# VITA-Group/mm-hand

Hardware: AMD Instinct MI355X
Metric: 256x256 hand images/sec (G+D step) (higher is better)
Workload: dtype f32; 1 GPU; RHD-shaped 256x256, per-GPU batch 32, fp32 (Winograd F(6x6,3x3) on the 3x3 stack), G(9 PATBlocks, ngf64)+D_PB+D_PP+L1/perceptual/GAN+Adam, --norm instance, dropout on; VGG19[:4] weights: random-init (seed 1234): NOT the reference's pretrained objective; global_batch=32, parallelism=dp1

## Files before the change

### include/mmhand_hip.h

```cpp
#ifndef MMHAND_HIP_H
#define MMHAND_HIP_H

#include <stddef.h>
#include <stdint.h>

#ifdef __cplusplus
extern "C" {
#endif
#pragma GCC visibility push(default)

typedef void* mmh_stream_t;

enum { MMH_PAD_ZERO = 0, MMH_PAD_REFLECT = 1 };
enum { MMH_ACT_NONE = 0, MMH_ACT_RELU = 1, MMH_ACT_TANH = 2 };
enum { MMH_F32 = 0, MMH_BF16 = 1, MMH_FP16 = 2 };

typedef struct mmh_conv_desc {
    int32_t B, H, W;
    int32_t Cin, Cout;
    int32_t kh, kw;
    int32_t stride;
    int32_t pad;
    int32_t pad_mode;
    int32_t Ho, Wo;
    int32_t x_cs, y_cs;
    int32_t dtype;
} mmh_conv_desc;

const char* mmh_last_error(void);
int mmh_version(void);
int mmh_set_option(const char* key, int value);
int mmh_get_option(const char* key, int* value);
const char* mmh_option_key(int index);


int mmh_conv2d_fprop(const mmh_conv_desc* d, const void* x, const void* w,
                     const void* bias, void* y, int act, mmh_stream_t s);

int mmh_conv2d_fprop_stats_chunks(const mmh_conv_desc* d);
int mmh_conv2d_fprop_stats(const mmh_conv_desc* d, const void* x, const void* w, const void* bias,
                           void* y, void* stats, mmh_stream_t s);
int mmh_dgrad_s2_halo_supported(const mmh_conv_desc* d, int dx_cs);

int mmh_conv2d_dgrad(const mmh_conv_desc* d, const void* dy, const void* w,
                     void* dx, int dx_cs, mmh_stream_t s);

size_t mmh_conv2d_dgrad_folded_ws_bytes(const mmh_conv_desc* d);
int mmh_conv2d_dgrad_folded(const mmh_conv_desc* d, const void* dy, const void* w,
                            void* dx, void* ws, size_t ws_bytes, mmh_stream_t s);

int mmh_wino_weights(const void* w, int Cin, int Cout, int flip_transpose, int tile, int dtype,
                     void* U, mmh_stream_t s);
int mmh_wino_input(const void* x, int B, int H, int W, int C, int reflect, int tile, int dtype,
                   void* V, mmh_stream_t s);
int mmh_wino_dy(const void* dy, int B, int H, int W, int C, int tile, int dtype, void* Yh,
                mmh_stream_t s);
int mmh_wino_input_dy(const void* dy, int B, int H, int W, int C, int tile, int dtype, void* V,
                      void* Yh, int fold, mmh_stream_t s);
int mmh_wino_gemm(const void* V, const void* U, void* M, int64_t tiles, int K, int N,
                  int nbatch, int dtype, mmh_stream_t s);
int mmh_wino_gemm_levels(const void* V, const void* U, void* M, int64_t tiles, int K, int N,
                         int nbatch, int levels, mmh_stream_t s);
int mmh_wino_gemm_levels16(const void* V, const void* U, void* M, int64_t tiles, int K, int N, int levels,
                           mmh_stream_t s);
int mmh_wino_weights_multi(const void* table, int n, int64_t total_blocks, mmh_stream_t s);
int mmh_wino_output(const void* M, void* y, const void* bias, int B, int H, int W, int C,
                    int act, int tile, int dtype, void* stats, int fold, mmh_stream_t s);
size_t mmh_wino_wgrad_gemm_ws_bytes(int64_t tiles, int Cin, int Cout, int nbatch);
int mmh_wino_wgrad_gemm(const void* V, const void* Yh, int64_t tiles, int Cin, int Cout,
                        int nbatch, int dtype, void* ws, size_t ws_bytes, void* dU,
                        mmh_stream_t s);
int mmh_wino_dw(const void* dU, int Cin, int Cout, int tile, void* dw, int accumulate,
                mmh_stream_t s);
size_t mmh_conv2d_dgrad_border_ws_bytes(const mmh_conv_desc* d);
int mmh_conv2d_dgrad_border(const mmh_conv_desc* d, const void* dy, const void* w, void* dx,
                            void* ws, size_t ws_bytes, int phase, int io16, mmh_stream_t s);

size_t mmh_conv2d_wgrad_ws_bytes(const mmh_conv_desc* d);
int mmh_conv2d_wgrad(const mmh_conv_desc* d, const void* x, const void* dy,
                     void* dw, void* ws, size_t ws_bytes, int accumulate,
                     int io16, mmh_stream_t s);

int mmh_convT2d_fprop(const mmh_conv_desc* d, const void* x, const void* w,
                      const void* bias, void* y, int y_cs, int act,
                      mmh_stream_t s);
int mmh_convT2d_dgrad(const mmh_conv_desc* d, const void* dy, const void* w,
                      void* dx, mmh_stream_t s);
int mmh_convT2d_wgrad(const mmh_conv_desc* d, const void* x, const void* dy,
                      void* dw, void* ws, size_t ws_bytes, int accumulate,
                     int io16, mmh_stream_t s);

int mmh_prep_weights_bf16(const void* w, int taps, int Cin, int Cout,
                          void* w_plain, void* w_t, mmh_stream_t s);
int mmh_prep_weights_fp16(const void* w, int taps, int Cin, int Cout,
                          void* w_plain, void* w_t, mmh_stream_t s);
// ... 438 lines not shown
```

### mmhand_amd/csrc/common.h

```cpp
#pragma once
#include <hip/hip_runtime.h>
#include <cstdarg>
#include <cstdio>
#include <cstdint>
#include "../../include/mmhand_hip.h"

namespace mmh {

char* err_buf();
int fail(const char* fmt, ...);

inline int check_launch(const char* what) {
    hipError_t e = hipGetLastError();
    if (e != hipSuccess) return fail("%s: %s", what, hipGetErrorString(e));
    return 0;
}

inline hipStream_t as_stream(mmh_stream_t s) { return reinterpret_cast<hipStream_t>(s); }

inline int64_t cdiv(int64_t a, int64_t b) { return (a + b - 1) / b; }

int wino6_weights(const float* w, float* U, int Cin, int Cout, int flip_transpose, hipStream_t st);
int wino6_weights_multi(const long long* table, int n, long long total_blocks, hipStream_t st);
int wino6_input(const float* x, float* V, int B, int H, int W, int C, int reflect, int xcd, hipStream_t st);
int wino6_output(const float* M, float* y, const float* bias, int B, int H, int W, int C, int act, float* stats,
                 int fold, hipStream_t st);
int wino6_dy(const float* dy, float* Yh, int B, int H, int W, int C, hipStream_t st);
int wino6_input_normact(const float* x, float* V, int B, int H, int W, int C, int reflect, int xcd,
                        const float* scale, const float* shift, int groups, int relu, float drop_p,
                        const uint32_t* drows, hipStream_t st);
int wino6_input_dy_normbwd(const float* g, const float* x, float* V, float* Yh, int B, int H, int W, int C, int xcd,
                           int fold, const float* mean, const float* invstd, const float* gamma, const float* s1,
                           const float* s2, double count, const float* scale, const float* shift,
                           const uint32_t* drows, int groups, int relu, float drop_p, hipStream_t st);
int wino6_input_dy(const float* dy, float* V, float* Yh, int B, int H, int W, int C, int xcd, int fold,
                   hipStream_t st);
int wino6_dw(const float* dU, float* dw, int Cin, int Cout, int accumulate, hipStream_t st);
bool wgrad_lp16t_supported(const mmh_conv_desc* d);
int wgrad_lp16t_splits(const mmh_conv_desc* d);
int launch_wgrad_lp16t(const mmh_conv_desc* d, const void* x16, const void* dy16, float* slab, const void* zeros,
                       hipStream_t st);
bool dgrad_s2_halo_ok(const mmh_conv_desc* d, int dx_cs, int act);
int launch_dgrad_s2_halo(const mmh_conv_desc* d, const void* dy, const void* w, const void* bias, void* dx, int dx_cs,
                         int act, hipStream_t st);
extern int g_dgrad_s2_halo, g_dgrad_s2_dbg;
bool wgrad_s2_strip_ok(const mmh_conv_desc* d);
size_t wgrad_s2_strip_ws_bytes(const mmh_conv_desc* d);
int launch_wgrad_s2_strip(const mmh_conv_desc* d, const void* x, const void* dy, void* dw, void* ws, size_t ws_bytes,
                          int accumulate, hipStream_t st);
extern int g_wgrad_s2_strip;
bool stem_f32_ok(const mmh_conv_desc* d);
int stem_f32_stats_chunks(const mmh_conv_desc* d);
int launch_stem_f32(const mmh_conv_desc* d, const void* x, const void* w, const void* bias, void* y, int act, float* stats,
                    hipStream_t st);
extern int g_stem_f32, g_stem_f32_dbg, g_stem_f32_levels;
extern int g_stem_sparse;
extern int g_stem_sparse_flat;
void wgrad_flat_split(int Mrows, int N, int P, int& splits, int& pix_per_split);
bool wino_wgrad_dma_ok(int64_t tiles, int Cin, int Cout, int nbatch);
size_t wino_wgrad_dma_ws_bytes(int64_t tiles, int Cin, int Cout, int nbatch);
int launch_wino_wgrad_dma(const float* V, const float* Yh, int64_t tiles, int Cin, int Cout, int nbatch, float* ws, float* dU,
                          hipStream_t st);
extern int g_wino_wgrad_dma;
int launch_slab_reduce(const float* slab, float* dw, int64_t n4_total, int splits, int accumulate, int64_t n4, hipStream_t st);
bool conv_s2f_ok(const mmh_conv_desc* d, int mode);
bool conv_s1f_ok(const mmh_conv_desc* d, int mode);
int conv_s2f_stats_chunks(const mmh_conv_desc* d);
int launch_conv_s2f(const mmh_conv_desc* d, const void* x16, const void* w16, const void* bias, void* y, int y_is16, int act,
                    const void* zeros, hipStream_t st, float* stats = nullptr, int mode = 0);
bool conv_s2d_ok(const mmh_conv_desc* d, int mode);
int launch_conv_s2d(const mmh_conv_desc* d, const void* g16, const void* w16, const void* bias, void* dx, int dx_is16, int act,
                    const void* zeros, hipStream_t st);
extern int g_lp16_s2f;
extern int g_lp16_persist;
extern int g_slab_reduce_par;
extern int g_wino6_vec;
extern int g_lp16_shape;
extern int g_lp16_tap_inner;
extern int g_lp16_dbg;
extern int g_lp16_wgrad_ring;
extern int g_lp16_wgrad_s2;
extern int g_pw_v2;
extern int g_col_chunks, g_row_chunks;

}

#define MMH_REQUIRE(cond, ...)                      \
    do {                                            \
        if (!(cond)) return mmh::fail(__VA_ARGS__); \
    } while (0)
```

### mmhand_amd/csrc/conv_igemm.hip

```cpp
#include <algorithm>
#include <cstring>
#include "device_prims.h"

namespace {
using namespace mmh::dev;

typedef __bf16 bf16x4 __attribute__((ext_vector_type(4)));
typedef __bf16 bf16x2 __attribute__((ext_vector_type(2)));
typedef _Float16 f16x4 __attribute__((ext_vector_type(4)));
typedef _Float16 f16x2 __attribute__((ext_vector_type(2)));
__device__ __forceinline__ bf16x4 to_bf16x4(float4 v) {
    bf16x4 r;
    r[0] = (__bf16)v.x; r[1] = (__bf16)v.y; r[2] = (__bf16)v.z; r[3] = (__bf16)v.w;
    return r;
}
template <bool H16>
__device__ __forceinline__ bf16x4 to_lp4(float4 v) {
    if (H16) {
        f16x4 r;
        r[0] = (_Float16)v.x; r[1] = (_Float16)v.y; r[2] = (_Float16)v.z; r[3] = (_Float16)v.w;
        return __builtin_bit_cast(bf16x4, r);
    }
    return to_bf16x4(v);
}
template <int LP>
__device__ __forceinline__ void wst4(void* base, long long idx4, float4 v) {
    if (LP) reinterpret_cast<bf16x4*>(base)[idx4] = to_lp4<LP == 2>(v);
    else reinterpret_cast<float4*>(base)[idx4] = v;
}
template <int LP>
__device__ __forceinline__ float4 wld4(const void* base, long long idx4) {
    if (LP == 2) {
        const f16x4 r = reinterpret_cast<const f16x4*>(base)[idx4];
        return make_float4((float)r[0], (float)r[1], (float)r[2], (float)r[3]);
    }
    if (LP == 1) {
        const bf16x4 r = reinterpret_cast<const bf16x4*>(base)[idx4];
        return make_float4((float)r[0], (float)r[1], (float)r[2], (float)r[3]);
    }
    return reinterpret_cast<const float4*>(base)[idx4];
}

constexpr int BM = 128;
constexpr int BK = 32;
constexpr int LDA = 36;
constexpr int LDW = 132;
constexpr int TABP = 8;
constexpr size_t tab_bytes(int rows) { return (size_t)rows * TABP * 2 * sizeof(int); }

struct Gather {
    const float* src;
    unsigned src_bytes;
    int srcH, srcW;
    unsigned src_cs;
    int PH, PW;
    int TH, TW;
    int C4;
    int ap_h, at_h, a0_h;
// ... 389 lines not shown
#pragma unroll
            for (int e = 0; e < 4; ++e) {
#pragma unroll
                for (int i = 0; i < TM; ++i) {
                    const float a = e == 0 ? av[i].x : e == 1 ? av[i].y : e == 2 ? av[i].z : av[i].w;
#pragma unroll
                    for (int j = 0; j < TN; ++j)
                        acc[i][j] = __builtin_amdgcn_mfma_f32_32x32x2f32(a, bsc[j][e], acc[i][j], 0, 0, 0);
                }
            }
        }
        }
        if (!(p.dbg & 2)) {
            if (!DBUF) __syncthreads();
            if (ks + 1 < p.nk) store_tiles(DBUF ? ((ks + 1) & 1) : 0);
            __syncthreads();
        }
    }

    float bv[TN];
#pragma unroll
    for (int j = 0; j < TN; ++j) {
        const int n = n0 + wn * WTN + j * 32 + l31;
        bv[j] = (p.bias && n < p.N) ? p.bias[n] : 0.f;
    }
#pragma unroll
    for (int i = 0; i < TM; ++i) {
#pragma unroll
        for (int r = 0; r < 16; ++r) {
            const int m = m0 + wm * WTM + i * 32 + (r & 3) + 8 * (r >> 2) + 4 * h;
            if (m >= p.M) continue;
            unsigned off;
            if (p.out_linear) off = (unsigned)m * p.out_cs;
            else {
                int b = m / PHW;
                int rr = m - b * PHW;
                int ph = rr / g.PW;
                int pw = rr - ph * g.PW;
                off = ((unsigned)(b * p.OH + ph * p.o_p + p.o0_h) * (unsigned)p.OW +
                       (unsigned)(pw * p.o_p + p.o0_w)) * p.out_cs;
            }
#pragma unroll
            for (int j = 0; j < TN; ++j) {
                const int n = n0 + wn * WTN + j * 32 + l31;
                if (n < p.N) {
                    float v = acc[i][j][r] + bv[j];
                    if (p.accum) v += p.out[off + n];
                    p.out[off + n] = act_apply(v, p.act);
                }
            }
        }
    }
    if (p.stats) {
        constexpr float CNT = (float)(TM * 16);
#pragma unroll
        for (int j = 0; j < TN; ++j) {
            const int n = n0 + wn * WTN + j * 32 + l31;
            const float b = (p.bias && n < p.N) ? p.bias[n] : 0.f;
            float sum = 0.f;
#pragma unroll
            for (int i = 0; i < TM; ++i)
#pragma unroll
                for (int r = 0; r < 16; ++r) sum += acc[i][j][r] + b;
            const float mean_l = sum * (1.f / CNT);
            float m2 = 0.f;
#pragma unroll
            for (int i = 0; i < TM; ++i)
#pragma unroll
                for (int r = 0; r < 16; ++r) {
                    const float dv = acc[i][j][r] + b - mean_l;
                    m2 += dv * dv;
                }
            const float mean_o = __shfl_xor(mean_l, 32, 64), m2_o = __shfl_xor(m2, 32, 64);
            const float dm = mean_o - mean_l;
            if (h == 0 && n < p.N) {
                float* o = p.stats + ((size_t)(mt * WAVES_M + wm) * 3) * p.N + n;
                o[0] = 2.f * CNT;
                o[p.N] = mean_l + 0.5f * dm;
                o[2 * p.N] = m2 + m2_o + dm * dm * (0.5f * CNT);
            }
        }
    }
}

template <int BN, int WAVES_M, int WAVES_N, bool B_NMAJOR, bool DBUF>
__global__ void __launch_bounds__(256, 2) conv_igemm_kernel(const ConvKP p) {
    conv_igemm_body<BN, WAVES_M, WAVES_N, B_NMAJOR, DBUF>(p, blockIdx.x, blockIdx.y, gridDim.x, gridDim.y);
}

__global__ void __launch_bounds__(256, 2) conv_igemm_levels2_kernel(const ConvKP p) {
    conv_igemm_body<128, 2, 2, false, false, 128, 2>(p, blockIdx.x, blockIdx.y, gridDim.x, gridDim.y);
}

__global__ void __launch_bounds__(256, 2) conv_igemm_dgrad_levels2_kernel(const ConvKP p) {
    conv_igemm_body<128, 2, 2, true, false, 128, 2>(p, blockIdx.x, blockIdx.y, gridDim.x, gridDim.y);
}

template <int BN, int WAVES_M, int WAVES_N, bool B_NMAJOR>
__global__ void __launch_bounds__(256, 2) conv_igemm_tall_kernel(const ConvKP p) {
    conv_igemm_body<BN, WAVES_M, WAVES_N, B_NMAJOR, false, 256>(p, blockIdx.x, blockIdx.y, gridDim.x, gridDim.y);
}

constexpr int MAXP = 9;
struct MultiKP {
    ConvKP p[MAXP];
    int start[MAXP + 1];
    int n;
};
__device__ __forceinline__ int multi_piece(const MultiKP& mp, int L) {
    int k = 0;
    while (k + 1 < mp.n && L >= mp.start[k + 1]) ++k;
    return k;
}
template <int BN, int WAVES_M, int WAVES_N, bool B_NMAJOR, int BMT = 128>
__global__ void __launch_bounds__(256, 2) conv_igemm_multi_kernel(const MultiKP mp) {
    const int k = multi_piece(mp, blockIdx.x);
    const ConvKP& p = mp.p[k];
    const int gx = (p.N + BN - 1) / BN, gy = (p.M + BMT - 1) / BMT;
    const int local = blockIdx.x - mp.start[k];
    conv_igemm_body<BN, WAVES_M, WAVES_N, B_NMAJOR, false, BMT>(p, local % gx, local / gx, gx, gy);
}

struct BatchKP {
    ConvKP p;
    long long src_bs, w_bs, out_bs;
};
template <int BN, int WAVES_M, int WAVES_N, bool B_NMAJOR>
__global__ void __launch_bounds__(256, 2) conv_igemm_batched_kernel(const BatchKP bp) {
    ConvKP p = bp.p;
    const long long z = blockIdx.z;
    p.g.src += z * bp.src_bs;
    p.w += z * bp.w_bs;
    p.out += z * bp.out_bs;
// ... 1424 lines not shown
__global__ void reflect_fold_kernel(const float* __restrict__ dxp, float* __restrict__ dx, int B,
                                    int H, int W, int C4, int p) {
    const int64_t total = (int64_t)B * H * W * C4;
    const int Hp = H + 2 * p, Wp = W + 2 * p;
    int64_t i = (int64_t)blockIdx.x * blockDim.x + threadIdx.x;
    const int64_t stride = (int64_t)gridDim.x * blockDim.x;
    for (; i < total; i += stride) {
        int c = (int)(i % C4);
        int64_t t = i / C4;
        int w = (int)(t % W); t /= W;
        int hh = (int)(t % H);
        int b = (int)(t / H);
        int hs[3], ws[3], nh = 0, nw = 0;
        hs[nh++] = hh;
        if (hh >= 1 && hh <= p) hs[nh++] = -hh;
        if (hh >= H - 1 - p && hh <= H - 2) hs[nh++] = 2 * (H - 1) - hh;
        ws[nw++] = w;
        if (w >= 1 && w <= p) ws[nw++] = -w;
        if (w >= W - 1 - p && w <= W - 2) ws[nw++] = 2 * (W - 1) - w;
        float4 s = make_float4(0.f, 0.f, 0.f, 0.f);
        for (int a = 0; a < nh; ++a)
            for (int e = 0; e < nw; ++e) {
                const float4 v = reinterpret_cast<const float4*>(
                    dxp)[(((int64_t)b * Hp + hs[a] + p) * Wp + ws[e] + p) * C4 + c];
                s.x += v.x; s.y += v.y; s.z += v.z; s.w += v.w;
            }
        reinterpret_cast<float4*>(dx)[i] = s;
    }
}

inline bool is16(int dtype) { return dtype == MMH_BF16 || dtype == MMH_FP16; }

int validate(const mmh_conv_desc* d) {
    MMH_REQUIRE(d != nullptr, "conv desc is NULL");
    MMH_REQUIRE(d->dtype == MMH_F32 || is16(d->dtype), "bad dtype=%d", d->dtype);
    MMH_REQUIRE(d->Cin % 4 == 0 && d->Cout % 4 == 0, "Cin/Cout must be multiples of 4 (%d,%d)",
                d->Cin, d->Cout);
    MMH_REQUIRE(d->x_cs % 4 == 0 && d->y_cs % 4 == 0 && d->x_cs >= d->Cin && d->y_cs >= d->Cout,
                "bad channel strides x_cs=%d y_cs=%d", d->x_cs, d->y_cs);
    MMH_REQUIRE(d->stride == 1 || d->stride == 2, "stride must be 1 or 2 (%d)", d->stride);
    MMH_REQUIRE(d->kh >= 1 && d->kw >= 1 && d->pad >= 0, "bad kernel/pad");
    MMH_REQUIRE(d->pad_mode == MMH_PAD_ZERO || (d->stride == 1 && d->pad < d->H && d->pad < d->W),
                "reflect padding needs stride 1 and pad < H,W");
    MMH_REQUIRE(d->Ho == (d->H + 2 * d->pad - d->kh) / d->stride + 1 &&
                    d->Wo == (d->W + 2 * d->pad - d->kw) / d->stride + 1,
                "Ho/Wo inconsistent with H,W,k,s,p");
    MMH_REQUIRE((int64_t)d->B * (d->H + 2 * d->pad) * (d->W + 2 * d->pad) * (int64_t)d->x_cs < (1ll << 30) &&
                    (int64_t)d->B * d->Ho * d->Wo * (int64_t)d->y_cs < (1ll << 30) &&
                    (int64_t)d->kh * d->kw * d->Cin * d->Cout < (1ll << 30),
                "tensor too large for 32-bit byte offsets (4 GiB per buffer)");
    return 0;
}

int g_conv_cw = 0;

void set_korder(Gather& g, int& nk, int& Kflat) {
    Kflat = g.TH * g.TW * g.C4 * 4;
    if (g.C4 % 8 == 0) {
        g.chunk_major = 1;
        nk = (g.C4 / 8) * g.TH * g.TW;
        const int chunks = g.C4 / 8;
        g.cw = (g_conv_cw > 0 && chunks % g_conv_cw == 0) ? g_conv_cw
               : (chunks % 2 == 0 ? 2 : 1);
    } else {
        g.chunk_major = 0; g.cw = 1; nk = (Kflat + BK - 1) / BK;
        g.dc4 = 8 % g.C4; g.dtw = (8 / g.C4) % g.TW; g.dth = (8 / g.C4) / g.TW;
    }
}

template <typename K>
int allow_lds(K kernel, size_t bytes) {
    hipError_t e = hipFuncSetAttribute(reinterpret_cast<const void*>(kernel),
                                       hipFuncAttributeMaxDynamicSharedMemorySize, (int)bytes);
    if (e != hipSuccess) return mmh::fail("hipFuncSetAttribute(LDS=%zu): %s", bytes, hipGetErrorString(e));
    return 0;
}

int g_conv_dbuf = 0;
int g_conv_dbg = 0;
int g_conv_xcd = 1;

template <int BN, int WM, int WN, bool NMAJOR, bool DBUF>
int launch_conv_t(const ConvKP& p, hipStream_t st) {
    constexpr size_t lds = (DBUF ? 2 : 1) * (BM * LDA + (NMAJOR ? BN * LDA : BK * BN)) * sizeof(float) + tab_bytes(BM);
    static int ready = -1;
    if (ready != 0) ready = allow_lds(conv_igemm_kernel<BN, WM, WN, NMAJOR, DBUF>, lds);
    if (ready != 0) return ready;
    dim3 grid((p.N + BN - 1) / BN, (p.M + BM - 1) / BM);
    hipLaunchKernelGGL((conv_igemm_kernel<BN, WM, WN, NMAJOR, DBUF>), grid, dim3(256), lds, st, p);
    return mmh::check_launch("conv_igemm_kernel");
}

template <int BN, int WM, int WN, bool NMAJOR>
int launch_conv_tall_t(const ConvKP& p, hipStream_t st) {
    constexpr size_t lds = (256 * LDA + (NMAJOR ? BN * LDA : BK * BN)) * sizeof(float) + tab_bytes(256);
    static int ready = -1;
    if (ready != 0) ready = allow_lds(conv_igemm_tall_kernel<BN, WM, WN, NMAJOR>, lds);
    if (ready != 0) return ready;
    dim3 grid((p.N + BN - 1) / BN, (p.M + 255) / 256);
    hipLaunchKernelGGL((conv_igemm_tall_kernel<BN, WM, WN, NMAJOR>), grid, dim3(256), lds, st, p);
    return mmh::check_launch("conv_igemm_tall_kernel");
}

template <int BN, int WM, int WN>
int launch_conv_bf16_t(const ConvKP& p, hipStream_t st) {
    constexpr size_t lds = (size_t)(BM + BN) * LDH * 2;
    static int ready = -1;
    if (ready != 0) ready = allow_lds(conv_igemm_bf16_kernel<BN, WM, WN>, lds);
// ... 66 lines not shown
    if (g_conv_levels == 2 && !NMAJOR && p.N > 64 && p.g.chunk_major) {
        const int gx = (p.N + 127) / 128, gy = (p.M + BM - 1) / BM;
        const_cast<ConvKP&>(p).xcd_remap = (g_conv_xcd && gx > 1 && gy >= 8) ? 1 : 0;
        return launch_conv_levels2(p, st);
    }
    if (g_conv_bn256 && !NMAJOR && p.N % 256 == 0) {
        const int gx = p.N / 256, gy = (p.M + BM - 1) / BM;
        const_cast<ConvKP&>(p).xcd_remap = (g_conv_xcd && gx > 1 && gy >= 8) ? 1 : 0;
        return launch_conv_t<256, 2, 2, NMAJOR, false>(p, st);
    }
    if (g_conv_tall == 2 && !p.stats && p.N > 32 && p.N <= 64 && p.M >= 256 * 512) {
        const_cast<ConvKP&>(p).xcd_remap = (g_conv_xcd1 && (p.M + 255) / 256 >= 8) ? 1 : 0;
        return launch_conv_tall_t<64, 4, 1, NMAJOR>(p, st);
    }
    {
        const int BNsel = p.N > 64 ? 128 : (p.N > 32 ? 64 : 32);
        const int gx = (p.N + BNsel - 1) / BNsel, gy = (p.M + BM - 1) / BM;
        const_cast<ConvKP&>(p).xcd_remap = (g_conv_xcd && (gx > 1 || g_conv_xcd1) && gy >= 8) ? 1 : 0;
    }
    if (p.N > 64)
        return g_conv_dbuf ? launch_conv_t<128, 2, 2, NMAJOR, true>(p, st)
                           : launch_conv_t<128, 2, 2, NMAJOR, false>(p, st);
    if (p.N > 32) return launch_conv_t<64, 2, 2, NMAJOR, false>(p, st);
    return launch_conv_t<32, 4, 1, NMAJOR, false>(p, st);
}

Gather fwd_gather(const mmh_conv_desc* d, const void* x) {
    Gather g{};
    g.src = static_cast<const float*>(x);
    g.src_bytes = (unsigned)((size_t)d->B * d->H * d->W * d->x_cs * sizeof(float));
    g.srcH = d->H; g.srcW = d->W; g.src_cs = (unsigned)d->x_cs;
    g.PH = d->Ho; g.PW = d->Wo;
    g.TH = d->kh; g.TW = d->kw;
    g.C4 = d->Cin / 4;
    g.ap_h = d->stride; g.at_h = 1; g.a0_h = -d->pad;
    g.ap_w = d->stride; g.at_w = 1; g.a0_w = -d->pad;
    g.shift = 0;
    g.reflect = d->pad_mode == MMH_PAD_REFLECT;
    return g;
}

int fprop_stats_chunks(const mmh_conv_desc* d) {
    if (mmh::stem_f32_ok(d)) return mmh::stem_f32_stats_chunks(d);
    const long long M = (long long)d->B * d->Ho * d->Wo;
    if (is16(d->dtype) || M % BM != 0 || d->Cout % 4 != 0) return 0;
    const int waves_m = d->Cout > 32 ? 2 : 4;
    return (int)(M / BM) * waves_m;
}

int do_fprop(const mmh_conv_desc* d, const void* x, const void* w, const void* bias, void* y,
             int act, hipStream_t st, float* stats = nullptr, const int* rect_pads = nullptr) {
    if (!rect_pads && mmh::stem_f32_ok(d) && (!stats || mmh::stem_f32_stats_chunks(d) > 0))
        return mmh::launch_stem_f32(d, x, w, bias, y, act, stats, st);
    ConvKP p{};
    p.stats = stats;
    p.g = fwd_gather(d, x);
    if (rect_pads) { p.g.a0_h = -rect_pads[0]; p.g.a0_w = -rect_pads[1]; }
    set_korder(p.g, p.nk, p.Kflat);
    p.w = static_cast<const float*>(w);
    p.w_bytes = (unsigned)((size_t)d->kh * d->kw * d->Cin * d->Cout * sizeof(float));
    p.out = static_cast<float*>(y);
    p.bias = static_cast<const float*>(bias);
    p.M = d->B * d->Ho * d->Wo;
    p.N = d->Cout;
    p.wCin = d->Cin; p.wCout = d->Cout;
    p.KW_true = d->kw; p.kh0 = 0; p.kw0 = 0; p.tstep = 1;
    p.out_linear = 1; p.out_cs = (unsigned)d->y_cs;
    p.OH = d->Ho; p.OW = d->Wo; p.o_p = 1;
    p.act = act;
    if (is16(d->dtype)) {
        p.h16 = d->dtype == MMH_FP16;
        if (d->Cin % 64 == 0) {
            p.wRows = d->Cout; p.wKper = d->Cin;
            p.w_bytes = (unsigned)((size_t)d->kh * d->kw * d->Cin * d->Cout * 2);
        } else {
            const int Kpad = (d->kh * d->kw * d->Cin + 63) / 64 * 64;
            p.flat16 = 1;
            p.wRows = d->Cout; p.wKper = Kpad;
            p.w_bytes = (unsigned)((size_t)d->Cout * Kpad * 2);
        }
        return launch_conv_bf16(p, st);
    }
    return launch_conv<false>(p, st);
}

int g_dgrad_s2_multi = 1;
template <int BN, int WM, int WN, int BMT = 128>
int launch_multi_t(MultiKP& mp, bool bf16, hipStream_t st);

int do_dgrad(const mmh_conv_desc* d, const void* dy, const void* w, const void* bias, void* dx,
             int dx_cs, int act, hipStream_t st) {
    const int s = d->stride;
    const int off = d->pad_mode == MMH_PAD_REFLECT ? d->pad : 0;
    const int OH = d->H + 2 * off, OW = d->W + 2 * off;
    MMH_REQUIRE(s == 1 || (OH % 2 == 0 && OW % 2 == 0), "stride-2 dgrad needs even H,W");
    if (mmh::dgrad_s2_halo_ok(d, dx_cs, act)) return mmh::launch_dgrad_s2_halo(d, dy, w, bias, dx, dx_cs, act, st);
    ConvKP classes[4];
    int ncls = 0;
    for (int ch = 0; ch < s; ++ch)
        for (int cw = 0; cw < s; ++cw) {
            const int kh0 = ((ch - off + d->pad) % s + s) % s;
            const int kw0 = ((cw - off + d->pad) % s + s) % s;
            const int TH = kh0 < d->kh ? (d->kh - kh0 + s - 1) / s : 0;
            const int TW = kw0 < d->kw ? (d->kw - kw0 + s - 1) / s : 0;
            ConvKP p{};
            Gather& g = p.g;
// ... 642 lines not shown
    p.slab = static_cast<float*>(ws);
    const bool bf16 = is16(d->dtype);
    p.h16 = d->dtype == MMH_FP16;
    p.pix_per_split = wgrad_pix_per_split(p.P, splits, bf16 ? BKP : BK);
    p.dbg = g_conv_dbg;
    p.nsplit = splits;
    int rc;
    if (bf16) {
        if (p.N > 64) rc = launch_wgrad_bf16_t<128, 2, 2>(p, splits, st);
        else if (p.N > 32) rc = launch_wgrad_bf16_t<64, 2, 2>(p, splits, st);
        else rc = launch_wgrad_bf16_t<32, 4, 1>(p, splits, st);
    } else if (g_wgrad_bn256 && p.N % 256 == 0) rc = launch_wgrad_t<256, 2, 2, false>(p, splits, st);
    else if (p.N > 64) rc = g_wgrad_dbuf ? launch_wgrad_t<128, 2, 2, true>(p, splits, st)
                                    : launch_wgrad_t<128, 2, 2, false>(p, splits, st);
    else if (p.N > 32) rc = launch_wgrad_t<64, 2, 2, false>(p, splits, st);
    else rc = launch_wgrad_t<32, 4, 1, false>(p, splits, st);
    if (rc) return rc;
    const int64_t n4 = (int64_t)p.Mrows * p.N / 4;
    return mmh::launch_slab_reduce(p.slab, static_cast<float*>(dw), n4, splits, accumulate, n4, st);
}

struct OptionEntry { const char* name; int* value; };
const OptionEntry* option_table(int* count) {
    static const OptionEntry table[] = {
        {"conv_dbuf", &g_conv_dbuf},
        {"conv_dbg", &g_conv_dbg},
        {"conv_cw", &g_conv_cw},
        {"conv_bn256", &g_conv_bn256},
        {"conv_levels", &g_conv_levels},
        {"dgrad_levels", &g_dgrad_levels},
        {"wino_bn256", &g_wino_bn256},
        {"conv_xcd", &g_conv_xcd},
        {"conv_xcd1", &g_conv_xcd1},
        {"conv_tall", &g_conv_tall},
        {"wgrad_slots", &g_wgrad_slots},
        {"wgrad_dbuf", &g_wgrad_dbuf},
        {"wgrad_bn256", &g_wgrad_bn256},
        {"wgrad_xcd", &g_wgrad_xcd},
        {"wino_wgrad_v2", &g_wino_wgrad_v2},
        {"wino_wgrad_occ", &g_wino_wgrad_occ},
        {"wino_gemm_v2", &g_wino_gemm_v2},
        {"wino_xcd", &g_wino_xcd},
        {"dgrad_s2_multi", &g_dgrad_s2_multi},
        {"wino6_vec", &mmh::g_wino6_vec},
        {"lp16_shape", &mmh::g_lp16_shape},
        {"lp16_s2f", &mmh::g_lp16_s2f},
        {"lp16_persist", &mmh::g_lp16_persist},
        {"lp16_tap_inner", &mmh::g_lp16_tap_inner},
        {"pw_v2", &mmh::g_pw_v2},
        {"col_chunks", &mmh::g_col_chunks},
        {"row_chunks", &mmh::g_row_chunks},
        {"dgrad_s2_halo", &mmh::g_dgrad_s2_halo},
        {"wgrad_s2_strip", &mmh::g_wgrad_s2_strip},
        {"stem_f32", &mmh::g_stem_f32},
        {"wino_wgrad_dma", &mmh::g_wino_wgrad_dma},
        {"stem_f32_dbg", &mmh::g_stem_f32_dbg},
        {"slab_reduce_par", &mmh::g_slab_reduce_par},
        {"dgrad_s2_dbg", &mmh::g_dgrad_s2_dbg},
        {"lp16_dbg", &mmh::g_lp16_dbg},
        {"lp16_wgrad_ring", &mmh::g_lp16_wgrad_ring},
        {"lp16_wgrad_s2", &mmh::g_lp16_wgrad_s2},
        {"border_bn64", &g_border_bn64},
        {"wino_gemm_occ", &g_wino_gemm_occ},
        {"wino_gemm_levels", &g_wino_gemm_levels},
        {"wino_gemm_bn", &g_wino_gemm_bn},
        {"wino_bf16_occ", &g_wino_bf16_occ},
        {"wino_bf16_bk", &g_wino_bf16_bk},
        {"wino_wgrad_bn256", &g_wino_wgrad_bn256},
        {"wino_wgrad_slots", &g_wino_wgrad_slots},
        {"stem_sparse", &mmh::g_stem_sparse},
        {"stem_sparse_flat", &mmh::g_stem_sparse_flat},
    };
    *count = (int)(sizeof(table) / sizeof(table[0]));
    return table;
}
const OptionEntry* find_option(const char* key) {
    int n = 0;
    const OptionEntry* t = option_table(&n);
    for (int i = 0; i < n; ++i)
        if (!strcmp(key, t[i].name)) return &t[i];
    return nullptr;
}

}

namespace mmh {
void wgrad_flat_split(int Mrows, int N, int P, int& splits, int& pix_per_split) {
    splits = wgrad_splits(Mrows, N, P);
    pix_per_split = wgrad_pix_per_split(P, splits, BK);
}
}

extern "C" {

int mmh_set_option(const char* key, int value) {
    MMH_REQUIRE(key != nullptr, "mmh_set_option: NULL key");
    const OptionEntry* e = find_option(key);
    if (!e) return mmh::fail("mmh_set_option: unknown key '%s'", key);
    if (e->value == &g_conv_levels) { g_conv_levels = value == 2 ? 2 : 1; mmh::g_stem_f32_levels = g_conv_levels; return 0; }
    if (e->value == &g_dgrad_levels) { g_dgrad_levels = value == 2 ? 2 : 1; return 0; }
    if (e->value == &mmh::g_col_chunks || e->value == &mmh::g_row_chunks)
        MMH_REQUIRE(value > 0, "mmh_set_option: '%s' needs a value > 0, got %d", key, value);
    *e->value = value;
    return 0;
}

// ... 504 lines not shown
```

### mmhand_amd/lib.py

```python
import ctypes as C
import os

_HERE = os.path.dirname(os.path.abspath(__file__))
LIB_PATH = os.environ.get("MMH_LIB_PATH") or os.path.join(_HERE, "libmmhand_hip.so")

PAD_ZERO, PAD_REFLECT = 0, 1
ACT_NONE, ACT_RELU, ACT_TANH = 0, 1, 2
F32, BF16, FP16 = 0, 1, 2
U8 = 3
POOL_MAX, POOL_AVG = 0, 1


class ConvDesc(C.Structure):
    _fields_ = [(n, C.c_int32) for n in (
        "B", "H", "W", "Cin", "Cout", "kh", "kw", "stride", "pad", "pad_mode",
        "Ho", "Wo", "x_cs", "y_cs", "dtype")]


class PlaneSrc(C.Structure):
    _fields_ = [("ptr", C.c_void_p), ("C", C.c_int32),
                ("sb", C.c_int64), ("sc", C.c_int64), ("sh", C.c_int64), ("sw", C.c_int64)]


class ImageSrc(C.Structure):
# ... 32 lines not shown
    "mmh_wino_weights_multi": (_i, [_vp, _i, _i64, _vp]),
    "mmh_prep_weights_lp16_multi": (_i, [_vp, _i, _i64, _vp]),
    "mmh_wino_output": (_i, [_vp, _vp, _vp, _i, _i, _i, _i, _i, _i, _i, _vp, _i, _vp]),
    "mmh_norm_stats_merge": (_i, [_vp, _i, _i, _i, _vp, _vp, _vp]),
    "mmh_norm_stats_merge2_ws_bytes": (_sz, [_i, _i]),
    "mmh_norm_stats_merge2": (_i, [_vp, _i, _i, _i, _vp, _sz, _vp, _vp, _vp]),
    "mmh_norm_stats_merge_finalize": (_i, [_vp, _i, _i, _i, _d, _f, _vp, _vp, _vp, _vp, _vp, _vp]),
    "mmh_wino_wgrad_gemm_ws_bytes": (_sz, [_i64, _i, _i, _i]),
    "mmh_wino_wgrad_gemm": (_i, [_vp, _vp, _i64, _i, _i, _i, _i, _vp, _sz, _vp, _vp]),
    "mmh_wino_dw": (_i, [_vp, _i, _i, _i, _vp, _i, _vp]),
    "mmh_conv2d_dgrad_border_ws_bytes": (_sz, [_DP]),
    "mmh_conv2d_dgrad_border": (_i, [_DP, _vp, _vp, _vp, _vp, _sz, _i, _i, _vp]),
    "mmh_conv7_thin_fprop": (_i, [_DP, _vp, _vp, _vp, _vp, _i, _vp]),
    "mmh_conv7_thin_dgrad_ws_bytes": (_sz, [_DP]),
    "mmh_conv7_thin_dgrad": (_i, [_DP, _vp, _vp, _vp, _vp, _sz, _i, _vp]),
    "mmh_conv7_thin_wgrad_ws_bytes": (_sz, [_DP]),
    "mmh_conv7_thin_wgrad": (_i, [_DP, _vp, _vp, _vp, _vp, _sz, _i, _vp]),
    "mmh_conv7_stem_wgrad_supported": (_i, [_DP]),
    "mmh_conv7_stem_wgrad_ws_bytes": (_sz, [_DP]),
    "mmh_conv7_stem_wgrad": (_i, [_DP, _vp, _vp, _vp, _vp, _sz, _i, _vp]),
    "mmh_stem_activity_bytes": (_sz, [_i, _i, _i]),
    "mmh_stem_activity": (_i, [_vp, _i, _i, _i, _i, _vp, _vp]),
    "mmh_conv7_stem_sparse_wgrad_flat_supported": (_i, [_DP]),
    "mmh_conv7_stem_sparse_wgrad_flat_ws_bytes": (_sz, [_DP]),
    "mmh_conv7_stem_sparse_wgrad_flat": (_i, [_DP, _vp, _vp, _vp, _vp, _vp, _sz, _i, _vp]),
    "mmh_conv7_stem_sparse_fprop_supported": (_i, [_DP]),
    "mmh_conv7_stem_sparse_fprop": (_i, [_DP, _vp, _vp, _vp, _vp, _vp, _vp, _vp]),
    "mmh_conv7_stem_sparse_wgrad_supported": (_i, [_DP]),
    "mmh_conv7_stem_sparse_wgrad_ws_bytes": (_sz, [_DP]),
    "mmh_conv7_stem_sparse_wgrad": (_i, [_DP, _vp, _vp, _vp, _vp, _vp, _sz, _i, _vp]),
    "mmh_conv2d_wgrad_ws_bytes": (_sz, [_DP]),
    "mmh_conv2d_wgrad": (_i, [_DP, _vp, _vp, _vp, _vp, _sz, _i, _i, _vp]),
    "mmh_convT2d_fprop": (_i, [_DP, _vp, _vp, _vp, _vp, _i, _i, _vp]),
    "mmh_convT2d_dgrad": (_i, [_DP, _vp, _vp, _vp, _vp]),
    "mmh_convT2d_wgrad": (_i, [_DP, _vp, _vp, _vp, _vp, _sz, _i, _i, _vp]),
    "mmh_reflect_fold": (_i, [_vp, _vp, _i, _i, _i, _i, _i, _vp]),
    "mmh_prep_weights_bf16": (_i, [_vp, _i, _i, _i, _vp, _vp, _vp]),
    "mmh_prep_weights_bf16_flat": (_i, [_vp, _i, _i, _i, _vp, _vp]),
    "mmh_prep_weights_fp16": (_i, [_vp, _i, _i, _i, _vp, _vp, _vp]),
    "mmh_prep_weights_fp16_flat": (_i, [_vp, _i, _i, _i, _vp, _vp]),
    "mmh_cvt_lp16": (_i, [_vp, _i64, _i, _vp, _vp]),
    "mmh_conv_lp16_supported": (_i, [_DP, _i]),
    "mmh_conv_lp16": (_i, [_DP, _i, _vp, _vp, _vp, _vp, _i, _i, _vp, _vp]),
    "mmh_conv_lp16_stats_chunks": (_i, [_DP]),
    "mmh_conv_lp16_fprop_stats": (_i, [_DP, _vp, _vp, _vp, _vp, _vp, _vp, _vp]),
    "mmh_conv_stem16_stats_chunks": (_i, [_DP, _i]),
    "mmh_conv_stem16_stats": (_i, [_DP, _vp, _i, _vp, _vp, _vp, _vp, _vp, _vp]),
    "mmh_lp16_pad_cvt": (_i, [_vp, _i64, _i, _i, _i, _vp, _vp]),
    "mmh_prep_weights_lp16_flat8": (_i, [_vp, _i, _i, _i, _i, _i, _vp, _vp]),
    "mmh_conv_lp16_flat_supported": (_i, [_DP, _i]),
    "mmh_conv_lp16_flat": (_i, [_DP, _vp, _i, _vp, _vp, _vp, _i, _i, _vp, _vp]),
    "mmh_conv_stem16_supported": (_i, [_DP, _i]),
    "mmh_dgrad_s2_halo_supported": (_i, [_DP, _i]),
    "mmh_conv_stem16_weights_bytes": (_sz, [_i]),
    "mmh_prep_weights_stem16": (_i, [_vp, _i, _i, _i, _vp, _vp]),
    "mmh_conv_stem16_weights_bytes_k": (_sz, [_i, _i]),
    "mmh_prep_weights_stem16_k": (_i, [_vp, _i, _i, _i, _i, _vp, _vp]),
    "mmh_conv_stem16": (_i, [_DP, _vp, _i, _vp, _vp, _vp, _i, _i, _vp, _vp]),
    "mmh_wgrad_stem_lp16_supported": (_i, [_DP, _i]),
    "mmh_wgrad_stem_lp16_ws_bytes": (_sz, [_DP, _i]),
    "mmh_wgrad_stem_lp16": (_i, [_DP, _vp, _i, _vp, _vp, _vp, _sz, _i, _vp, _vp]),
    "mmh_conv7_head_wgrad_lp16_supported": (_i, [_DP]),
    "mmh_conv7_head_wgrad_lp16_ws_bytes": (_sz, [_DP]),
    "mmh_conv7_head_wgrad_lp16": (_i, [_DP, _vp, _vp, _vp, _vp, _sz, _i, _vp, _vp]),
    "mmh_wgrad_lp16_flat_supported": (_i, [_DP, _i]),
    "mmh_wgrad_lp16_flat_ws_bytes": (_sz, [_DP, _i]),
    "mmh_wgrad_lp16_flat": (_i, [_DP, _vp, _i, _i, _vp, _vp, _vp, _sz, _i, _vp, _vp]),
    "mmh_conv7_head_dgrad_lp16_supported": (_i, [_DP]),
    "mmh_conv7_head_dgrad_lp16_ws_bytes": (_sz, [_DP]),
    "mmh_conv7_head_dgrad_lp16": (_i, [_DP, _vp, _vp, _vp, _i, _vp, _sz, _vp, _vp]),
    "mmh_conv7_n4_lp16_supported": (_i, [_DP, _i]),
    "mmh_conv7_n4_lp16_ws_bytes": (_sz, [_DP, _i]),
    "mmh_conv7_n4_lp16": (_i, [_DP, _i, _vp, _vp, _vp, _vp, _i, _vp, _sz, _vp, _vp]),
    "mmh_conv3x3_lp16_supported": (_i, [_DP]),
    "mmh_conv3x3_lp16_fold_supported": (_i, [_DP]),
    "mmh_wgrad3x3_lp16_ws_bytes": (_sz, [_DP]),
    "mmh_wgrad3x3_lp16": (_i, [_DP, _vp, _vp, _vp, _vp, _sz, _i, _vp, _vp]),
    "mmh_conv3x3_lp16": (_i, [_DP, _i, _vp, _vp, _vp, _vp, _i, _i, _vp, _vp]),
    "mmh_conv3x3_lp16_stats_chunks": (_i, [_DP]),
    "mmh_conv3x3_lp16_dgrad_nbr_chunks": (_i, [_DP, _i]),
    "mmh_conv3x3_lp16_dgrad_nbr": (_i, [_DP, _i, _vp, _vp, _vp, _vp, _vp, _vp, _vp, _i, _f, _vp, _vp, _vp, _sz, _vp, _vp]),
    "mmh_norm_bwd_sums_final": (_i, [_vp, _i, _i, _i, _vp, _vp, _vp]),
    "mmh_conv3x3_lp16_dgrad_add_supported": (_i, [_DP]),
    "mmh_conv3x3_lp16_dgrad_add": (_i, [_DP, _i, _vp, _vp, _vp, _vp, _vp, _vp]),
    "mmh_conv3x3_lp16_fprop_stats": (_i, [_DP, _vp, _vp, _vp, _vp, _vp, _vp, _vp]),
    "mmh_colsum_ws_bytes": (_sz, [_i64, _i]),
    "mmh_colsum": (_i, [_vp, _i64, _i, _i, _vp, _vp, _sz, _i, _i, _vp]),
    "mmh_norm_stats_ws_bytes": (_sz, [_i, _i64, _i]),
    "mmh_norm_stats": (_i, [_vp, _i, _i64, _i, _i, _vp, _vp, _vp, _sz, _i, _vp]),
    "mmh_norm_finalize": (_i, [_vp, _vp, _d, _vp, _vp, _f, _i, _i, _vp, _vp, _vp, _vp, _vp, _f, _vp]),
    "mmh_syncbn_merge_finalize": (_i, [_vp, _i, _i64, _i, _d, _f, _vp, _vp, _vp, _vp, _vp, _vp, _vp, _vp, _vp, _f, _vp]),
    "mmh_scale_shift_act": (_i, [_vp, _vp, _vp, _vp, _vp, _i, _i64, _i, _i, _f, _u64, _vp, _vp, _i, _i, _vp]),
    "mmh_scale_shift_act_twin": (_i, [_vp, _vp, _vp, _vp, _vp, _i, _i64, _i, _i, _f, _u64, _vp, _vp, _i, _i, _vp, _i, _vp]),
    "mmh_norm_bwd_ws_bytes": (_sz, [_i, _i64, _i]),
    "mmh_norm_bwd_reduce": (_i, [_vp, _vp, _vp, _vp, _vp, _i, _i64, _i, _i, _f, _vp, _vp, _vp, _sz, _i, _i, _vp]),
    "mmh_norm_bwd_apply": (_i, [_vp, _vp, _vp, _vp, _vp, _vp, _vp, _vp, _d, _i, _i64, _i, _i, _f, _vp, _i, _i, _i, _vp]),
    "mmh_norm_bwd_fused_supported": (_i, [_i, _i64, _i, _i, _i, _i]),
    "mmh_norm_bwd_fused": (_i, [_vp, _vp, _vp, _vp, _vp, _vp, _d, _i, _i64, _i, _i, _f, _vp, _vp, _vp, _i, _i, _i, _vp]),
    "mmh_dropout_bits": (_i, [_i64, _f, _u64, _vp, _vp, _vp]),
    "mmh_dropout_bits_rows": (_i, [_vp, _i64, _i, _i, _vp, _vp]),
    "mmh_dropout_bits_both": (_i, [_i64, _i, _i, _f, _u64, _vp, _vp, _vp, _vp]),
    "mmh_norm_bwd_reduce_rc": (_i, [_vp, _vp, _vp, _vp, _vp, _vp, _vp, _i, _i64, _i, _i, _f, _vp, _vp, _vp, _sz, _vp]),
    "mmh_norm_bwd_apply_rc": (_i, [_vp, _vp, _vp, _vp, _vp, _vp, _vp, _vp, _vp, _vp, _d, _i, _i64, _i, _i, _f, _vp, _vp]),
    "mmh_wino_input_normact": (_i, [_vp, _i, _i, _i, _i, _i, _vp, _vp, _vp, _i, _i, _f, _vp, _vp]),
    "mmh_wino_input_dy_normbwd": (_i, [_vp, _vp, _i, _i, _i, _i, _vp, _vp, _i, _vp, _vp, _vp, _vp, _vp, _d, _vp, _vp,
                                       _vp, _i, _i, _f, _vp]),
# ... 126 lines not shown
```

Baseline: 130.1 images/s.

## Add persistent LDS-pipelined fp32 MFMA kernel for stride-2 3x3 downsampling convs

Adds a dedicated persistent kernel for the two stride-2 3x3 zero-pad encoder convs (64->128, 128->256) in fp32. Each workgroup loops over output tiles, streaming input rows and weight slices into LDS through a double-buffered ring of async DMA copies, and accumulates with 32x32x2 f32 MFMA. It fuses bias, activation and instance-norm column statistics into the epilogue. The stats reduction is moved into a shared header so the generic igemm path uses the same code. The aim is to replace the generic gather-based implicit GEMM for these layers with better data reuse and load/compute overlap, at the cost of a large, shape-specific kernel with hand-tuned wait counts.

```diff
diff --git a/include/mmhand_hip.h b/include/mmhand_hip.h
--- a/include/mmhand_hip.h
+++ b/include/mmhand_hip.h
@@ -41,6 +41,7 @@
 int mmh_conv2d_fprop_stats(const mmh_conv_desc* d, const void* x, const void* w, const void* bias,
                            void* y, void* stats, mmh_stream_t s);
 int mmh_dgrad_s2_halo_supported(const mmh_conv_desc* d, int dx_cs);
+int mmh_fprop_s2_supported(const mmh_conv_desc* d);
 
 int mmh_conv2d_dgrad(const mmh_conv_desc* d, const void* dy, const void* w,
                      void* dx, int dx_cs, mmh_stream_t s);
diff --git a/mmhand_amd/csrc/common.h b/mmhand_amd/csrc/common.h
--- a/mmhand_amd/csrc/common.h
+++ b/mmhand_amd/csrc/common.h
@@ -44,6 +44,11 @@
 int launch_dgrad_s2_halo(const mmh_conv_desc* d, const void* dy, const void* w, const void* bias, void* dx, int dx_cs,
                          int act, hipStream_t st);
 extern int g_dgrad_s2_halo, g_dgrad_s2_dbg;
+bool fprop_s2_ok(const mmh_conv_desc* d);
+int launch_fprop_s2(const mmh_conv_desc* d, const void* x, const void* w, const void* bias, void* y, int act, float* stats,
+                    hipStream_t st);
+extern int g_fprop_s2, g_fprop_s2_wgs;
+extern int g_conv_cw;
 bool wgrad_s2_strip_ok(const mmh_conv_desc* d);
 size_t wgrad_s2_strip_ws_bytes(const mmh_conv_desc* d);
 int launch_wgrad_s2_strip(const mmh_conv_desc* d, const void* x, const void* dy, void* dw, void* ws, size_t ws_bytes,
diff --git a/mmhand_amd/csrc/conv_igemm.hip b/mmhand_amd/csrc/conv_igemm.hip
--- a/mmhand_amd/csrc/conv_igemm.hip
+++ b/mmhand_amd/csrc/conv_igemm.hip
@@ -1,9 +1,13 @@
 #include <algorithm>
 #include <cstring>
 #include "device_prims.h"
+#include "fprop_stats.h"
+
+namespace mmh { int g_conv_cw = 0; }
 
 namespace {
 using namespace mmh::dev;
+using mmh::g_conv_cw;
 
 typedef __bf16 bf16x4 __attribute__((ext_vector_type(4)));
 typedef __bf16 bf16x2 __attribute__((ext_vector_type(2)));
@@ -499,33 +503,11 @@
         }
     }
     if (p.stats) {
-        constexpr float CNT = (float)(TM * 16);
 #pragma unroll
         for (int j = 0; j < TN; ++j) {
             const int n = n0 + wn * WTN + j * 32 + l31;
             const float b = (p.bias && n < p.N) ? p.bias[n] : 0.f;
-            float sum = 0.f;
-#pragma unroll
-            for (int i = 0; i < TM; ++i)
-#pragma unroll
-                for (int r = 0; r < 16; ++r) sum += acc[i][j][r] + b;
-            const float mean_l = sum * (1.f / CNT);
-            float m2 = 0.f;
-#pragma unroll
-            for (int i = 0; i < TM; ++i)
-#pragma unroll
-                for (int r = 0; r < 16; ++r) {
-                    const float dv = acc[i][j][r] + b - mean_l;
-                    m2 += dv * dv;
-                }
-            const float mean_o = __shfl_xor(mean_l, 32, 64), m2_o = __shfl_xor(m2, 32, 64);
-            const float dm = mean_o - mean_l;
-            if (h == 0 && n < p.N) {
-                float* o = p.stats + ((size_t)(mt * WAVES_M + wm) * 3) * p.N + n;
-                o[0] = 2.f * CNT;
-                o[p.N] = mean_l + 0.5f * dm;
-                o[2 * p.N] = m2 + m2_o + dm * dm * (0.5f * CNT);
-            }
+            fprop_col_stats<TM, TN>(&acc[0][j], b, h, n < p.N, p.stats + ((size_t)(mt * WAVES_M + wm) * 3) * p.N + n, p.N);
         }
     }
 }
@@ -2056,8 +2038,6 @@
     return 0;
 }
 
-int g_conv_cw = 0;
-
 void set_korder(Gather& g, int& nk, int& Kflat) {
     Kflat = g.TH * g.TW * g.C4 * 4;
     if (g.C4 % 8 == 0) {
@@ -2230,6 +2210,7 @@
              int act, hipStream_t st, float* stats = nullptr, const int* rect_pads = nullptr) {
     if (!rect_pads && mmh::stem_f32_ok(d) && (!stats || mmh::stem_f32_stats_chunks(d) > 0))
         return mmh::launch_stem_f32(d, x, w, bias, y, act, stats, st);
+    if (!rect_pads && mmh::fprop_s2_ok(d)) return mmh::launch_fprop_s2(d, x, w, bias, y, act, stats, st);
     ConvKP p{};
     p.stats = stats;
     p.g = fwd_gather(d, x);
@@ -2978,6 +2959,8 @@
         {"row_chunks", &mmh::g_row_chunks},
         {"dgrad_s2_halo", &mmh::g_dgrad_s2_halo},
         {"wgrad_s2_strip", &mmh::g_wgrad_s2_strip},
+        {"fprop_s2", &mmh::g_fprop_s2},
+        {"fprop_s2_wgs", &mmh::g_fprop_s2_wgs},
         {"stem_f32", &mmh::g_stem_f32},
         {"wino_wgrad_dma", &mmh::g_wino_wgrad_dma},
         {"stem_f32_dbg", &mmh::g_stem_f32_dbg},
diff --git a/mmhand_amd/csrc/fprop_s2.hip b/mmhand_amd/csrc/fprop_s2.hip
--- /dev/null
+++ b/mmhand_amd/csrc/fprop_s2.hip
@@ -0,0 +1,266 @@
+#include <algorithm>
+#include <type_traits>
+#include <utility>
+#include "device_prims.h"
+#include "fprop_stats.h"
+
+namespace mmh { int g_fprop_s2 = 1; int g_fprop_s2_wgs = 0; }
+
+namespace {
+using namespace mmh::dev;
+
+constexpr int NT = 512;
+constexpr int UPX = 64;
+constexpr int XPX = 2 * UPX + 1;
+constexpr int PIXB = 256;
+constexpr int ENT_P = (XPX * PIXB + 1023) / 1024;
+constexpr int ENT_B = ENT_P * 1024;
+constexpr int XPIECES = 2 * ENT_P;
+constexpr int XROUNDS = (XPIECES + 7) / 8;
+constexpr int X_B = 4 * ENT_B;
+constexpr int WST_B = NT * 16;
+constexpr int LDS_B = X_B + 3 * WST_B;
+
+__device__ char g_zero_line[128];
+constexpr int wait_vm(int n) { return (n & 15) | ((n >> 4) << 14) | 0x0070; }
+template <int V> using IC = std::integral_constant<int, V>;
+template <typename F, int... J>
+__device__ __forceinline__ void unrolled(F& f, std::integer_sequence<int, J...>) { (f(IC<J>{}), ...); }
+
+struct FpropS2KP {
+    const float* x;
+    const float* w;
+    const float* bias;
+    float* y;
+    float* stats;
+    int H, W, Ho, Wo, x_cs, y_cs, act;
+    int tiles;
+};
+
+template <int CIN>
+__global__ void __launch_bounds__(NT, 1) fprop_s2_kernel(const FpropS2KP p) {
+    constexpr int N = 2 * CIN;
+    constexpr int R = WST_B / 4 / N;
+    constexpr int KGS = R / 8;
+    constexpr int SPC = 64 / R;
+    constexpr int SPP = 3 * SPC;
+    constexpr int NPH = 3 * (CIN / 64);
+    constexpr int SPT = NPH * SPP;
+    constexpr int TN = N / 128;
+    static_assert(SPP % 3 == 0 && SPP >= XROUNDS + 3, "the ring slot of a stage and the wait counts are per-phase constants");
+    extern __shared__ __attribute__((aligned(1024))) char smem[];
+    const int tid = threadIdx.x;
+    const int lane = tid & 63, wave = __builtin_amdgcn_readfirstlane(tid >> 6);
+    const int l31 = lane & 31, h = lane >> 5;
+    const int u = wave >> 2, cg = wave & 3;
+    const unsigned lds0 = lds_addr_of(smem);
+    const unsigned wdst = __builtin_amdgcn_readfirstlane(lds0 + (unsigned)wave * 1024u);
+
+    const int G = gridDim.x;
+    const int L = (G & 7) ? (int)blockIdx.x : (int)((blockIdx.x & 7) * (G >> 3) + (blockIdx.x >> 3));
+    const int t0 = (int)((long long)L * p.tiles / G), t1 = (int)((long long)(L + 1) * p.tiles / G);
+    const int nphase = (t1 - t0) * NPH;
+    if (nphase <= 0) return;
+    const int HoWo = p.Ho * p.Wo;
+
+    int x_off[XROUNDS];
+    int x_kind[XROUNDS];
+#pragma unroll
+    for (int r = 0; r < XROUNDS; ++r) {
+        const int q = 8 * r + wave;
+        const int local = (q >= ENT_P ? q - ENT_P : q) * 64 + lane;
+        const int px = local >> 4, cpos = local & 15;
+        x_off[r] = (px - 1) * p.x_cs + ((cpos ^ ((px >> 1) & 15)) << 2);
+        x_kind[r] = px >= XPX ? 2 : (px == 0 ? 1 : 0);
+    }
+    const void* const zero = g_zero_line + (lane & 7) * 16;
+    const float* xb[2];
+    bool xleft[2];
+    auto x_phase = [&](int g) {
+        const bool live = g < nphase;
+        const int tile = t0 + g / NPH, pi = g % NPH;
+        const int c = pi / 3, kh = pi - 3 * c;
+#pragma unroll
+        for (int uu = 0; uu < 2; ++uu) {
+            const int m = tile * 128 + UPX * uu;
+            const int b = m / HoWo, rem = m - b * HoWo;
+            const int ph = rem / p.Wo, pw0 = rem - ph * p.Wo;
+            const int row = 2 * ph - 1 + kh;
+            const bool ok = live && row >= 0;
+            xb[uu] = ok ? p.x + ((size_t)(b * p.H + row) * p.W + 2 * pw0) * (size_t)p.x_cs + c * 64 : nullptr;
+            xleft[uu] = pw0 > 0;
+        }
+    };
+    auto issue_x = [&](int r, int buf) {
+        const int q = 8 * r + wave;
+        if (q < XPIECES) {
+            const int uu = q >= ENT_P ? 1 : 0;
+            const bool ok = xb[uu] != nullptr && (x_kind[r] == 0 || (x_kind[r] == 1 && xleft[uu]));
+            const void* g = ok ? (const void*)(xb[uu] + x_off[r]) : zero;
+            lds_dma16(g, wdst + (unsigned)(buf * 2 * ENT_B) + (unsigned)(r * 8 * 1024));
+        }
+    };
+    auto issue_w = [&](int s, int slot) {
+        int row0;
+        if (CIN == 64) row0 = s * R;
+        else {
+            const int tc = s / SPC, wi = s - tc * SPC;
+            const int c = tc / 9, tap = tc - 9 * c;
+            row0 = tap * CIN + c * 64 + wi * R;
+        }
+        dma16_s(p.w + (size_t)row0 * N, (unsigned)tid * 16u, wdst + (unsigned)(X_B + slot * WST_B));
+    };
+
+    unsigned a_lane[2][3];
+#pragma unroll
+    for (int i = 0; i < 2; ++i)
+#pragma unroll
+        for (int kw = 0; kw < 3; ++kw) {
+            const int px = 2 * (32 * i + l31) + kw;
+            a_lane[i][kw] = lds0 + (unsigned)(u * ENT_B + px * PIXB) + (unsigned)((h ^ ((px >> 1) & 15)) << 4);
+        }
+    const int ncol = cg * 32 * TN + l31;
+    const unsigned b_lane = lds0 + (unsigned)X_B + (unsigned)((4 * h * N + ncol) * 4);
+    float bv[TN];
+#pragma unroll
+    for (int j = 0; j < TN; ++j) {
+        bv[j] = p.bias ? p.bias[ncol + 32 * j] : 0.f;
+        asm volatile("" : "+v"(bv[j]));
+    }
+
+    f32x16 acc[2][TN];
+#pragma unroll
+    for (int i = 0; i < 2; ++i)
+#pragma unroll
+        for (int j = 0; j < TN; ++j)
+#pragma unroll
+            for (int r = 0; r < 16; ++r) acc[i][j][r] = 0.f;
+
+    x_phase(0);
+#pragma unroll
+    for (int r = 0; r < XROUNDS; ++r) issue_x(r, 0);
+    issue_w(0, 0);
+    issue_w(1, 1);
+    int s_next = 2 % SPT;
+
+    for (int g = 0; g < nphase; ++g) {
+        const int buf = g & 1;
+        const unsigned xbuf = (unsigned)(buf * 2 * ENT_B);
+        auto stage = [&](auto jc) {
+            constexpr int j = decltype(jc)::value;
+            constexpr int kw = j / SPC, wi = j - SPC * (j / SPC), slot = j % 3;
+            constexpr int behind = 1 + ((j >= 2 && j - 2 < XROUNDS - 1) ? 1 : 0) + ((j >= 1 && j - 1 < XROUNDS - 1) ? 1 : 0);
+            asm volatile("" ::: "memory");
+            __builtin_amdgcn_s_waitcnt(wait_vm(behind));
+            __builtin_amdgcn_s_barrier();
+            asm volatile("" ::: "memory");
+            issue_w(s_next, (j + 2) % 3);
+            s_next = s_next + 1 == SPT ? 0 : s_next + 1;
+            if (j == 0) x_phase(g + 1);
+            if (j < XROUNDS) issue_x(j, buf ^ 1);
+#pragma unroll
+            for (int kgl = 0; kgl < KGS; ++kgl) {
+                const int kc = wi * KGS + kgl;
+                f32x4 af[2];
+#pragma unroll
+                for (int i = 0; i < 2; ++i) af[i] = lds_f4((a_lane[i][kw] + xbuf) ^ (unsigned)(kc << 5));
+                float bf[TN][4];
+#pragma unroll
+                for (int jn = 0; jn < TN; ++jn)
+#pragma unroll
+                    for (int e = 0; e < 4; ++e) bf[jn][e] = lds_f(b_lane, slot * WST_B + ((8 * kgl + e) * N + 32 * jn) * 4);
+#pragma unroll
+                for (int e = 0; e < 4; ++e)
+#pragma unroll
+                    for (int i = 0; i < 2; ++i)
+#pragma unroll
+                        for (int jn = 0; jn < TN; ++jn)
+                            acc[i][jn] = __builtin_amdgcn_mfma_f32_32x32x2f32(af[i][e], bf[jn][e], acc[i][jn], 0, 0, 0);
+            }
+        };
+        unrolled(stage, std::make_integer_sequence<int, SPP>{});
+
+        if ((g + 1) % NPH == 0) {
+            const int tile = t0 + g / NPH;
+            const int mu = tile * 128 + UPX * u;
+#pragma unroll
+            for (int i = 0; i < 2; ++i)
+#pragma unroll
+                for (int r = 0; r < 16; ++r) {
+                    float* const o = p.y + (size_t)(mu + 32 * i + (r & 3) + 8 * (r >> 2) + 4 * h) * (size_t)p.y_cs + ncol;
+#pragma unroll
+                    for (int j = 0; j < TN; ++j) o[32 * j] = act_apply(acc[i][j][r] + bv[j], p.act);
+                }
+            if (p.stats) {
+#pragma unroll
+                for (int j = 0; j < TN; ++j)
+                    fprop_col_stats<2, TN>(&acc[0][j], bv[j], h, true, p.stats + ((size_t)(tile * 2 + u) * 3) * N + ncol + 32 * j, N);
+            }
+#pragma unroll
+            for (int i = 0; i < 2; ++i)
+#pragma unroll
+                for (int j = 0; j < TN; ++j)
+#pragma unroll
+                    for (int r = 0; r < 16; ++r) acc[i][j][r] = 0.f;
+        }
+    }
+    asm volatile("s_waitcnt vmcnt(0)" ::: "memory");
+}
+
+int device_cus() {
+    static int cus = 0;
+    if (!cus) {
+        int dev = 0;
+        hipDeviceProp_t prop;
+        if (hipGetDevice(&dev) != hipSuccess || hipGetDeviceProperties(&prop, dev) != hipSuccess) return 0;
+        cus = prop.multiProcessorCount;
+    }
+    return cus;
+}
+
+template <int CIN>
+int launch_t(const FpropS2KP& p, int wgs, hipStream_t st) {
+    static int ready = -1;
+    if (ready != 0) {
+        hipError_t e = hipFuncSetAttribute(reinterpret_cast<const void*>(fprop_s2_kernel<CIN>),
+                                           hipFuncAttributeMaxDynamicSharedMemorySize, LDS_B);
+        if (e != hipSuccess) return mmh::fail("fprop_s2: %s", hipGetErrorString(e));
+        ready = 0;
+    }
+    hipLaunchKernelGGL((fprop_s2_kernel<CIN>), dim3(wgs), dim3(NT), LDS_B, st, p);
+    return mmh::check_launch("fprop_s2_kernel");
+}
+
+}
+
+namespace mmh {
+
+bool fprop_s2_ok(const mmh_conv_desc* d) {
+    return g_fprop_s2 && g_stem_f32_levels != 2 && g_conv_cw == 0 && d->dtype == MMH_F32 && d->kh == 3 && d->kw == 3 &&
+           d->stride == 2 && d->pad == 1 && d->pad_mode == MMH_PAD_ZERO &&
+           ((d->Cin == 64 && d->Cout == 128) || (d->Cin == 128 && d->Cout == 256)) && d->H % 2 == 0 && d->W % 2 == 0 &&
+           d->H == 2 * d->Ho && d->W == 2 * d->Wo && d->Wo % UPX == 0 && ((long long)d->B * d->Ho * d->Wo) % 128 == 0 &&
+           d->x_cs >= d->Cin && d->x_cs % 4 == 0 && d->y_cs >= d->Cout &&
+           (size_t)d->B * d->H * d->W * d->x_cs < (1ull << 31) && (size_t)d->B * d->Ho * d->Wo * d->y_cs < (1ull << 31);
+}
+
+int launch_fprop_s2(const mmh_conv_desc* d, const void* x, const void* w, const void* bias, void* y, int act, float* stats,
+                    hipStream_t st) {
+    FpropS2KP p{};
+    p.x = static_cast<const float*>(x);
+    p.w = static_cast<const float*>(w);
+    p.bias = static_cast<const float*>(bias);
+    p.y = static_cast<float*>(y);
+    p.stats = stats;
+    p.H = d->H; p.W = d->W; p.Ho = d->Ho; p.Wo = d->Wo; p.x_cs = d->x_cs; p.y_cs = d->y_cs; p.act = act;
+    p.tiles = (int)((long long)d->B * d->Ho * d->Wo / 128);
+    const int cus = device_cus();
+    if (cus <= 0) return fail("fprop_s2: cannot query the device");
+    int wgs = std::min(p.tiles, cus);
+    if (g_fprop_s2_wgs > 0) wgs = std::min(wgs, g_fprop_s2_wgs);
+    return d->Cin == 64 ? launch_t<64>(p, wgs, st) : launch_t<128>(p, wgs, st);
+}
+
+}
+
+extern "C" int mmh_fprop_s2_supported(const mmh_conv_desc* d) { return d && mmh::fprop_s2_ok(d) ? 1 : 0; }
diff --git a/mmhand_amd/csrc/fprop_stats.h b/mmhand_amd/csrc/fprop_stats.h
--- /dev/null
+++ b/mmhand_amd/csrc/fprop_stats.h
@@ -0,0 +1,32 @@
+#pragma once
+#include "device_prims.h"
+
+namespace mmh { namespace dev {
+
+template <int TM, int STRIDE>
+__device__ __forceinline__ void fprop_col_stats(const f32x16* acc0, float b, int h, bool ok, float* o, int N) {
+    constexpr float CNT = (float)(TM * 16);
+    float sum = 0.f;
+#pragma unroll
+    for (int i = 0; i < TM; ++i)
+#pragma unroll
+        for (int r = 0; r < 16; ++r) sum += acc0[i * STRIDE][r] + b;
+    const float mean_l = sum * (1.f / CNT);
+    float m2 = 0.f;
+#pragma unroll
+    for (int i = 0; i < TM; ++i)
+#pragma unroll
+        for (int r = 0; r < 16; ++r) {
+            const float dv = acc0[i * STRIDE][r] + b - mean_l;
+            m2 += dv * dv;
+        }
+    const float mean_o = __shfl_xor(mean_l, 32, 64), m2_o = __shfl_xor(m2, 32, 64);
+    const float dm = mean_o - mean_l;
+    if (h == 0 && ok) {
+        o[0] = 2.f * CNT;
+        o[N] = mean_l + 0.5f * dm;
+        o[2 * N] = m2 + m2_o + dm * dm * (0.5f * CNT);
+    }
+}
+
+} }
diff --git a/mmhand_amd/lib.py b/mmhand_amd/lib.py
--- a/mmhand_amd/lib.py
+++ b/mmhand_amd/lib.py
@@ -108,6 +108,7 @@
     "mmh_conv_lp16_flat": (_i, [_DP, _vp, _i, _vp, _vp, _vp, _i, _i, _vp, _vp]),
     "mmh_conv_stem16_supported": (_i, [_DP, _i]),
     "mmh_dgrad_s2_halo_supported": (_i, [_DP, _i]),
+    "mmh_fprop_s2_supported": (_i, [_DP]),
     "mmh_conv_stem16_weights_bytes": (_sz, [_i]),
     "mmh_prep_weights_stem16": (_i, [_vp, _i, _i, _i, _vp, _vp]),
     "mmh_conv_stem16_weights_bytes_k": (_sz, [_i, _i]),
```

Result: no change. 130.2 images/s (median of 2 runs) (+0.0%).
